# parthjaggi/flow

Measured on AMD Instinct MI355X. Metric: env-steps/sec, higher is better.
Workload: dtype mixed

## Files before the change

### flow_amd/build.py

```python
import concurrent.futures
import hashlib
import os
import shutil
import subprocess

PKG = os.path.dirname(os.path.abspath(__file__))
ROOT = os.path.dirname(PKG)
CSRC = os.path.join(PKG, "csrc")
SRC = os.path.join(CSRC, "flowsim.hip")
PART = os.path.join(CSRC, "flowsim_part.hip")
OBJ = os.path.join(CSRC, "_obj")
LIB = os.path.join(PKG, "libflowsim.so")

VALIDATED_ROCM = "7.2"

HEADERS = ["flowsim_sim.h", "flowsim_launch.h", "flowsim_kernels.h", "flowsim_open.h", "flowsim_wide.h",
           "flowsim_pair.h", "flowsim_pair_step_a.inc", "flowsim_pair_step_a_sm.inc", "flowsim_fig8.h", "flowsim_ringrl.h", "flowsim_policy.h", "flowsim_queue.h", "flowsim_queue_consts.h", "flowsim_dropq.h",
           "flowsim_learn.h",
           "flowsim_part.hip"]
DEPS = [SRC] + [os.path.join(CSRC, h) for h in HEADERS] + [os.path.join(ROOT, "include", "flowsim.h")]
assert all(os.path.exists(d) for d in DEPS)
_known = set(os.path.basename(d) for d in DEPS)
assert all(f in _known for f in os.listdir(CSRC) if f.endswith((".h", ".inc", ".hip"))), "flow_amd/build.py: a source under csrc/ is not in DEPS"

COMMON_FLAGS = ["--offload-arch=gfx950", "-O3", "-ffp-contract=off", "-std=c++17", "-Wall", "-Wno-unused-function"]
HIPCC_FLAGS = COMMON_FLAGS + ["-fPIC", "-shared"]


def parts():
    out = [("main", SRC, [])]
    for t, tn in (("float", "f32"), ("double", "f64")):
        for seg in (8, 16, 32, 64):
            out.append(("seg%d_%s" % (seg, tn), PART, ["-DFS_PART_T=" + t, "-DFS_PART_SEG=%d" % seg]))
        for w in (2, 4):
            out.append(("wide%d_%s" % (w, tn), PART, ["-DFS_PART_T=" + t, "-DFS_PART_WIDE=%d" % w]))
    out.append(("queue_f32", PART, ["-DFS_PART_T=float", "-DFS_PART_QUEUE=1"] +
                (["-DFS_QDIAG=1"] if os.environ.get("FLOWSIM_QDIAG") else [])))
    out.append(("learn_f32", PART, ["-DFS_PART_T=float", "-DFS_PART_LEARN=1"]))
    return out


def find_hipcc():
    for cand in (os.environ.get("HIPCC"), shutil.which("hipcc"), "/opt/rocm/bin/hipcc"):
        if cand and os.path.exists(cand):
            return cand
    raise RuntimeError("hipcc not found: libflowsim.so cannot be built (no CPU fallback exists)")


def include_flags():
    return ["-I" + os.path.join(ROOT, "include"), "-I" + CSRC]


def _stamp(extra):
    h = hashlib.sha256()
    for d in DEPS:
        h.update(os.path.relpath(d, ROOT).encode())
        with open(d, "rb") as f:
            h.update(hashlib.sha256(f.read()).digest())
# ... 158 lines not shown
```

### flow_amd/csrc/flowsim.hip

```cpp
#include "flowsim_sim.h"
#include "flowsim_learn.h"

namespace fsim {

int validate(const fs_config* c) {
  if (!c) return fail(FS_ERR_INVALID, "fs_create: cfg is NULL");
  if (c->struct_size != sizeof(fs_config))
    return fail(FS_ERR_INVALID, "fs_create: struct_size mismatch (header/library out of sync)");
  if (c->abi_version != FS_ABI_VERSION) return fail(FS_ERR_INVALID, "fs_create: abi_version mismatch");
  if (c->precision != FS_F32 && c->precision != FS_F64 && c->precision != FS_MIXED && c->precision != FS_F16S)
    return fail(FS_ERR_INVALID, "fs_create: bad precision");
  if (c->precision == FS_F16S && (c->network != FS_NET_MERGE || c->num_vehicles > 64))
    return fail(FS_ERR_UNSUPPORTED, "fs_create: FS_F16S (half state, float32 integrator) is built for FS_NET_MERGE "
                                    "(k_steps_open, <= 64 vehicle slots)");
  if (c->precision == FS_MIXED && (c->network == FS_NET_MERGE || c->network == FS_NET_BOTTLENECK)) {
  } else if (c->precision == FS_MIXED) {
    const bool fig8 = c->network == FS_NET_FIGURE_EIGHT;
    const char* why = nullptr;
    if ((c->network != FS_NET_RING && !fig8) || c->num_lanes > 1) why = "network (single-lane ring or figure eight)";
    else if (c->env != FS_ENV_ACCEL && c->env != FS_ENV_WAVE_ATTENUATION_PO) why = "env (AccelEnv or WaveAttenuationPOEnv)";
    else if (c->evaluate) why = "evaluate";
    else if (c->sims_per_step != 1) why = "sims_per_step (1)";
    else if (c->integrator != FS_EULER) why = "integrator (Euler)";
    else if (c->junction_mode && !fig8) why = "junction_mode";
// ... 214 lines not shown
    s->init_alive.assign(cfg->init_alive, cfg->init_alive + size_t(cfg->num_replicas) * cfg->num_vehicles);
    if (cfg->env == FS_ENV_BOTTLENECK_DV) {
      s->obs_cells.assign(cfg->obs_cells, cfg->obs_cells + cfg->num_obs_cells);
      if (cfg->num_rl > 0) s->act_cells.assign(cfg->act_cells, cfg->act_cells + cfg->num_rl);
    }
  }
  s->obs_dim = (cfg->env == FS_ENV_WAVE_ATTENUATION_PO) ? 3
               : (cfg->env == FS_ENV_WAVE_ATTENUATION_PO_MA) ? 3 * cfg->num_rl
               : (cfg->env == FS_ENV_ACCEL_PO_MA) ? 6 * cfg->num_rl
               : (cfg->env == FS_ENV_BOTTLENECK_DV) ? 4 * cfg->num_obs_cells + 1
               : (cfg->env == FS_ENV_BOTTLENECK) ? 1
               : (cfg->env == FS_ENV_MERGE_PO || cfg->env == FS_ENV_MERGE_MA)
                     ? 5 * cfg->num_rl
                     : (cfg->env == FS_ENV_LANE_CHANGE_ACCEL_PO)
                           ? (4 * (cfg->num_lanes < 1 ? 1 : cfg->num_lanes) + 1) * cfg->num_rl
                           : (cfg->env == FS_ENV_LANE_CHANGE_ACCEL ? 3 : 2) * cfg->num_vehicles;
  if (s->obs_dim < 1) s->obs_dim = 1;
  s->act_dim = cfg->num_rl * ((cfg->env == FS_ENV_LANE_CHANGE_ACCEL || cfg->env == FS_ENV_LANE_CHANGE_ACCEL_PO) ? 2 : 1);
  int seg = 8;
  while (seg < cfg->num_vehicles) seg <<= 1;
  s->seg = seg;
  hipError_t e = hipSetDevice(cfg->device);
  if (e == hipSuccess) e = hipStreamCreateWithFlags(&s->own_stream, hipStreamNonBlocking);
  if (e != hipSuccess) {
    delete s;
    return fail(FS_ERR_HIP, std::string("fs_create: no usable HIP device: ") + hipGetErrorString(e));
  }
  s->stream = s->own_stream;
  {
    const std::pair<const char*, bool SimBase::*> switches[] = {
        {"FLOWSIM_FORCE_GENERIC", &SimBase::force_generic}, {"FLOWSIM_NO_FASTDIV", &SimBase::no_fastdiv},
        {"FLOWSIM_NO_LOOP_KERNEL", &SimBase::no_loop_kernel}, {"FLOWSIM_NO_LOOP_FULL", &SimBase::no_loop_full},
        {"FLOWSIM_NO_RING_RL", &SimBase::no_ring_rl}, {"FLOWSIM_NO_QUEUE", &SimBase::no_queue},
        {"FLOWSIM_NO_PAIR", &SimBase::no_pair}, {"FLOWSIM_NO_MASK_SKIP", &SimBase::no_mask_skip}};
    for (const auto& sw : switches) {
      const char* v = std::getenv(sw.first);
      s->*sw.second = v && v[0] == '1';
    }
  }
  int rc = s->init();
  if (rc == FS_OK) {
    hipError_t e2 = hipStreamSynchronize(s->stream);
    if (e2 != hipSuccess) rc = fail(FS_ERR_HIP, std::string("fs_create: ") + hipGetErrorString(e2));
  }
  if (rc != FS_OK) {
    for (void* p : s->allocs) (void)hipFree(p);
    (void)hipStreamDestroy(s->own_stream);
    delete s;
    return rc;
  }
  s->cfg.vehicles = nullptr;
  s->cfg.ring_length = nullptr;
  s->cfg.init_pos = nullptr;
  s->cfg.init_vel = nullptr;
  s->cfg.init_lane = nullptr;
  s->cfg.segments = nullptr;
  s->cfg.inflows = nullptr;
  s->cfg.init_alive = nullptr;
  s->cfg.obs_cells = nullptr;
  s->cfg.obs_perm = nullptr;
  s->cfg.act_cells = nullptr;
  *out = reinterpret_cast<fs_handle>(static_cast<SimBase*>(s));
  return FS_OK;
}

inline SimBase* S(fs_handle h) { return reinterpret_cast<SimBase*>(h); }

// ... 338 lines not shown
```

### flow_amd/csrc/flowsim_kernels.h

```cpp
#pragma once
#include <hip/hip_runtime.h>
#include <stdint.h>

#include "flowsim.h"

namespace fs {

enum : int {
  FLAG_NEED_FOLLOWER = 1,
  FLAG_NEED_MEAN = 2,
  FLAG_HAS_NOISE = 4,
  FLAG_HAS_LAC = 8,
  FLAG_NEED_SUMO = 16,
  FLAG_HAS_FAILSAFE = 32,
  FLAG_ALL_IDM = 64,
  FLAG_IDM_SET = 128,
  FLAG_NO_FLOW_CTRL = 256,
  FLAG_DELTA4 = 512,
};

template <typename T>
struct DevView {
  T* pos;
  T* vel;
// ... 216 lines not shown
  T prv = dpp<DPP_WAVE_SHR1>(v);
  T last = v;
#pragma unroll
  for (int sg = 0; sg < 64 / SEG; ++sg) {
    T f = read_lane(v, sg * SEG + N - 1);
    last = (seg == sg) ? f : last;
  }
  return wrap ? last : prv;
}

template <int SEG, typename T>
__device__ __forceinline__ T seg_sum(T v) {
  v = v + dpp<DPP_QUAD_XOR1>(v);
  v = v + dpp<DPP_QUAD_XOR2>(v);
  v = v + dpp<DPP_ROW_HALF_MIRROR>(v);
  if (SEG >= 16) v = v + dpp<DPP_ROW_MIRROR>(v);
  if (SEG >= 32) v = add_swap16(v);
  if (SEG >= 64) v = add_swap32(v);
  return v;
}


template <int SHL, int SHR, typename T>
__device__ __forceinline__ T tr_combine(T lo, T hi, bool upper) {
  const T t = lo + dpp<SHL>(lo);
  const T u = hi + dpp<SHR>(hi);
  return upper ? u : t;
}
__device__ __forceinline__ float tr_combine16(float lo, float hi) {
  unsigned a = __builtin_bit_cast(unsigned, lo), b = __builtin_bit_cast(unsigned, hi);
  swap_rows16(a, b);
  return __builtin_bit_cast(float, a) + __builtin_bit_cast(float, b);
}
__device__ __forceinline__ double tr_combine16(double lo, double hi) {
  const unsigned long long bl = __builtin_bit_cast(unsigned long long, lo), bh = __builtin_bit_cast(unsigned long long, hi);
  unsigned l0 = unsigned(bl), l1 = unsigned(bl >> 32), h0 = unsigned(bh), h1 = unsigned(bh >> 32);
  swap_rows16(l0, h0);
  swap_rows16(l1, h1);
  return __builtin_bit_cast(double, ((unsigned long long)l1 << 32) | l0) +
         __builtin_bit_cast(double, ((unsigned long long)h1 << 32) | h0);
}
template <int SEG, int K, typename T>
__device__ __forceinline__ T transposed_sum(T* a, int lane) {
  static_assert(K <= 32 && K <= SEG, "at most min(SEG, 32) vectors");
  if (K >= 2) {
#pragma unroll
    for (int k = 0; k < K / 2; ++k) a[k] = tr_combine<DPP_ROW_SHL1, DPP_ROW_SHR1>(a[2 * k], a[2 * k + 1], (lane & 1) != 0);
  }
  if (K >= 4) {
#pragma unroll
    for (int k = 0; k < K / 4; ++k) a[k] = tr_combine<DPP_ROW_SHL2, DPP_ROW_SHR2>(a[2 * k], a[2 * k + 1], (lane & 2) != 0);
  }
  if (K >= 8) {
#pragma unroll
    for (int k = 0; k < K / 8; ++k) a[k] = tr_combine<DPP_ROW_SHL4, DPP_ROW_SHR4>(a[2 * k], a[2 * k + 1], (lane & 4) != 0);
  }
  if (K >= 16) {
#pragma unroll
    for (int k = 0; k < K / 16; ++k) a[k] = tr_combine<DPP_ROW_SHL8, DPP_ROW_SHR8>(a[2 * k], a[2 * k + 1], (lane & 8) != 0);
  }
  if (K >= 32) a[0] = tr_combine16(a[0], a[1]);
  T v = a[0];
  if (K < 2 && SEG >= 2) v = v + dpp<DPP_QUAD_XOR1>(v);
  if (K < 4 && SEG >= 4) v = v + dpp<DPP_QUAD_XOR2>(v);
  if (K < 8 && SEG >= 8) {
    if (K == 1) v = v + dpp<DPP_ROW_HALF_MIRROR>(v);
// ... 1446 lines not shown
```

### flow_amd/csrc/flowsim_launch.h

```cpp
#pragma once
#include "flowsim_sim.h"
#ifdef FS_PART_QUEUE
#include "flowsim_queue.h"
#include "flowsim_dropq.h"
#endif

namespace fsim {

#ifdef FS_PART_QUEUE
  template <typename T>
  int Sim<T>::launch_queue(const StepArgs& a) {
    const bool po = dv.env == FS_ENV_MERGE_PO;
    const bool noise = (dv.flags & fs::FLAG_HAS_NOISE) != 0, act = a.actions != nullptr && (po || ov.ma_apply_actions != 0);
    const auto k = pick(noise, [&](auto NZ) {
      return pick(act, [&](auto ACT) {
        return pick(po, [&](auto PO) { return &fs::k_merge_queue<NZ, ACT, false, PO>; });
      });
    });
    last_kernel = "k_merge_queue";
    hipLaunchKernelGGL(k, dim3(dv.R), dim3(64), 0, stream, dv, ov, qc, a.num_steps, a.actions, a.act_stride, a.obs, a.rew,
                       a.done, a.obs_every_step, fs::PolicyView{}, static_cast<float*>(nullptr), static_cast<float*>(nullptr),
                       0);
    return launched();
  }
// ... 202 lines not shown
                          : delta4 ? &fs::k_rollout_idm<T, SEG, true, false, BC> : &fs::k_rollout_idm<T, SEG, false, false, BC>;
    });
    last_kernel = "k_rollout_idm";
    const int waves = (dv.R + RPW - 1) / RPW;
    hipLaunchKernelGGL(k, dim3((waves + 7) / 8), dim3(512), 0, stream, dv, a.num_steps, a.obs, a.rew, a.done, d_dump);
    return launched();
  }

  template <typename T>
  template <int SEG>
  int Sim<T>::launch_k_steps(const StepArgs& a) {
    constexpr int RPW = 64 / SEG;
    auto k = &fs::k_steps<T, SEG, 0, 0>;
    last_kernel = "k_steps";
    if (fast_ok(a)) {
      k = &fs::k_steps<T, SEG, 1, 0>;
      last_kernel = "k_steps<FAST>";
    } else if ((dv.flags & fs::FLAG_IDM_SET) && !force_generic) {
      k = &fs::k_steps<T, SEG, 0, 1>;
      last_kernel = "k_steps<CSET>";
    }
    hipLaunchKernelGGL(k, dim3((dv.R + RPW - 1) / RPW), dim3(64), 0, stream, dv, a.num_steps, a.mask, a.actions,
                       a.act_stride, a.obs, a.rew, a.done, a.obs_every_step);
    return launched();
  }

  template <typename T>
  int Sim<T>::launch_policy_act(const fs::PolicyView& pv, int n_ag, const float* obs_in, float* act, float* logp) {
    last_kernel = "k_policy_act";
    const bool merge = dv.env == FS_ENV_MERGE_MA;
    hipLaunchKernelGGL(fs::k_policy_act<16>, dim3((dv.R * 16 + 255) / 256), dim3(256), 0, stream, pv, dv.R, n_ag, dv.rep0,
                       obs_in, act, logp, merge ? static_cast<const int*>(dv.lane) : nullptr,
                       merge ? static_cast<const int*>(dv.ctrl) : nullptr,
                       merge ? static_cast<const int*>(dv.rl_index) : nullptr, dv.N);
    return launched();
  }

  template <typename T>
  int Sim<T>::launch_policy_row16(const fs::PolicyView& pv, int num_steps, int reset_done, float* obs, float* act,
                                  float* logp, float* rew, uint8_t* done) {
    const bool fast = ringrl_fast_ok();
    auto kernel = [&](auto H) {
      return pick(dv.flags & fs::FLAG_HAS_NOISE, [&](auto NZ) {
        return pick(fast, [&](auto FA) { return &fs::k_ring_policy<T, H, NZ, FA>; });
      });
    };
    auto k = kernel(Int<1>());
    last_kernel = "k_ring_policy";
    if constexpr (std::is_same<T, float>::value) {
      if (dv.env == FS_ENV_WAVE_ATTENUATION_PO_MA) {
        k = kernel(Int<2>());
        last_kernel = "k_ring_policy<POMA>";
      }
    }
    const int waves = (dv.R + 3) / 4;
    hipLaunchKernelGGL(k, dim3((waves + 3) / 4), dim3(256), 0, stream, dv, pv, num_steps, reset_done, cfg.warmup_steps,
                       obs, act, logp, rew, done);
    return launched();
  }

  template <typename T>
  int Sim<T>::launch_policy_loop16(const fs::PolicyView& pv, int num_steps, int reset_done, float* obs, float* act,
                                   float* logp, float* rew, uint8_t* done) {
    if constexpr (std::is_same<T, float>::value) {
      const bool fastc = loop_delta4 && loop_fastc_ok();
      auto kernel = [&](auto H) {
        return fastc ? &fs::k_loop_policy<H, true, true>
// ... 16 lines not shown
```

### flow_amd/csrc/flowsim_policy.h

```cpp
#pragma once
#include "flowsim_ringrl.h"

namespace fs {

struct PolicyView {
  const float* w;
  const float* log_std;
  uint32_t* ctr;
  int in_dim, num_hidden, n_out;
  uint32_t seed_lo, seed_hi;
};

struct alignas(16) PolicyLds {
  float w_hid[2][16][16][4];
  float w_in[32][4];
  float w_wide[16][16][4];
  float b[3][32];
  float w_out[2][32];
  float b_out[2];
  float obs[4][4][4];
};

__host__ __device__ constexpr int policy_half(int in_dim) { return (in_dim + 1) >> 1; }

__device__ __forceinline__ void policy_wide_inputs(const float* o, int in_dim, int j, float& ia, float& ib) {
  const int half = policy_half(in_dim);
  ia = j < half ? o[j < half ? j : 0] : 0.0f;
  ib = (j < half && half + j < in_dim) ? o[half + j < in_dim ? half + j : 0] : 0.0f;
}

__device__ __forceinline__ const float* policy_load_trunk(const PolicyView& pv, PolicyLds* L, int tid, int nthreads) {
  const float* p = pv.w;
  const bool wide = pv.in_dim > 4;
  for (int e = tid; e < 32 * 4; e += nthreads) L->w_in[e / 4][e % 4] = (!wide && (e % 4) < pv.in_dim) ? p[(e / 4) * pv.in_dim + (e % 4)] : 0.0f;
  {
    const int half = policy_half(pv.in_dim);
    for (int e = tid; e < 32 * 32; e += nthreads) {
      const int u = e / 32, ip = e % 32;
      const int i = ip < 16 ? ip : half + (ip - 16);
      const bool used = wide && (ip & 15) < half && i < pv.in_dim;
      L->w_wide[ip >> 1][u & 15][(ip & 1) * 2 + (u >> 4)] = used ? p[u * pv.in_dim + i] : 0.0f;
    }
  }
  p += 32 * pv.in_dim;
  for (int e = tid; e < 32; e += nthreads) L->b[0][e] = p[e];
  p += 32;
  for (int l = 0; l < 2; ++l) {
    const bool have = l + 1 < pv.num_hidden;
    for (int e = tid; e < 32 * 32; e += nthreads) {
      const int u = e / 32, i = e % 32;
      L->w_hid[l][i >> 1][u & 15][(i & 1) * 2 + (u >> 4)] = have ? p[e] : 0.0f;
    }
    if (have) p += 32 * 32;
    for (int e = tid; e < 32; e += nthreads) L->b[l + 1][e] = have ? p[e] : 0.0f;
    if (have) p += 32;
  }
  return p;
}

__device__ __forceinline__ void policy_load(const PolicyView& pv, PolicyLds* L, int tid, int nthreads) {
  const float* p = policy_load_trunk(pv, L, tid, nthreads);
  for (int e = tid; e < 2 * 32; e += nthreads) L->w_out[e / 32][e % 32] = (e / 32) < pv.n_out ? p[e] : 0.0f;
  p += pv.n_out * 32;
  if (tid < 2) L->b_out[tid] = tid < pv.n_out ? p[tid] : 0.0f;
  __syncthreads();
}

template <int D1, int D2>
__device__ __forceinline__ void row_bcast(int k, float a, float b, float c, float& oa, float& ob, float& oc) {
#define FS_RB(K_) case K_: oa = dpp<DPP_ROW_NEWBCAST0 + K_>(a); ob = dpp<DPP_ROW_NEWBCAST0 + ((K_ + D1) & 15)>(b); \
                          oc = dpp<DPP_ROW_NEWBCAST0 + ((K_ + D2) & 15)>(c); break;
  switch (k & 15) {
    FS_RB(0) FS_RB(1) FS_RB(2) FS_RB(3) FS_RB(4) FS_RB(5) FS_RB(6) FS_RB(7)
    FS_RB(8) FS_RB(9) FS_RB(10) FS_RB(11) FS_RB(12) FS_RB(13) FS_RB(14) FS_RB(15)
  }
#undef FS_RB
}

__device__ __forceinline__ float policy_tanh(float z) {
  const float e = __builtin_amdgcn_exp2f(z * 2.885390081777927f);
  const float r = __builtin_amdgcn_rcpf(e + 1.0f);
  return __builtin_fmaf(-2.0f, r, 1.0f);
}

__device__ __forceinline__ f2 policy_layer(const float4 (&ww)[16], float b_j, float b_j16, float a, float b) {
  f2 z0 = {b_j, b_j16}, z1 = {0.0f, 0.0f}, z2 = {0.0f, 0.0f}, z3 = {0.0f, 0.0f};
  static_for<4>([&](auto q_c) {
    constexpr int q = decltype(q_c)::value;
    const float a0 = dpp<DPP_ROW_NEWBCAST0 + 4 * q>(a), a1 = dpp<DPP_ROW_NEWBCAST0 + 4 * q + 1>(a);
    const float a2 = dpp<DPP_ROW_NEWBCAST0 + 4 * q + 2>(a), a3 = dpp<DPP_ROW_NEWBCAST0 + 4 * q + 3>(a);
    const float b0 = dpp<DPP_ROW_NEWBCAST0 + 4 * q>(b), b1 = dpp<DPP_ROW_NEWBCAST0 + 4 * q + 1>(b);
    const float b2 = dpp<DPP_ROW_NEWBCAST0 + 4 * q + 2>(b), b3 = dpp<DPP_ROW_NEWBCAST0 + 4 * q + 3>(b);
    z0 = fma2(f2{ww[2 * q].x, ww[2 * q].y}, splat(a0), z0);
    z1 = fma2(f2{ww[2 * q].z, ww[2 * q].w}, splat(a1), z1);
    z2 = fma2(f2{ww[2 * q + 1].x, ww[2 * q + 1].y}, splat(a2), z2);
    z3 = fma2(f2{ww[2 * q + 1].z, ww[2 * q + 1].w}, splat(a3), z3);
    z0 = fma2(f2{ww[8 + 2 * q].x, ww[8 + 2 * q].y}, splat(b0), z0);
    z1 = fma2(f2{ww[8 + 2 * q].z, ww[8 + 2 * q].w}, splat(b1), z1);
    z2 = fma2(f2{ww[8 + 2 * q + 1].x, ww[8 + 2 * q + 1].y}, splat(b2), z2);
    z3 = fma2(f2{ww[8 + 2 * q + 1].z, ww[8 + 2 * q + 1].w}, splat(b3), z3);
  });
  return pk_add(pk_add(z0, z1), pk_add(z2, z3));
}

template <bool WIDE, bool PRE = false>
__device__ __forceinline__ void policy_trunk(const PolicyView& pv, const PolicyLds* L, int j, float o0, float o1, float o2,
                                             float& ha, float& hb) {
  float4 wa0 = make_float4(0.0f, 0.0f, 0.0f, 0.0f), wa1 = wa0;
  auto load_ahead = [&](int l) {
    wa0 = *reinterpret_cast<const float4*>(L->w_hid[l][0][j]);
    wa1 = *reinterpret_cast<const float4*>(L->w_hid[l][1][j]);
  };
  if (pv.num_hidden > 1) load_ahead(0);
  if constexpr (PRE) {
    ha = policy_tanh(o0);
    hb = policy_tanh(o1);
  } else if constexpr (WIDE) {
    float4 ww[16];
#pragma unroll
    for (int q = 0; q < 16; ++q) ww[q] = *reinterpret_cast<const float4*>(L->w_wide[q][j]);
    const f2 z = policy_layer(ww, L->b[0][j], L->b[0][j + 16], o0, o1);
    ha = policy_tanh(z.x);
    hb = policy_tanh(z.y);
  } else {
    const float4 wa = *reinterpret_cast<const float4*>(L->w_in[j]), wb = *reinterpret_cast<const float4*>(L->w_in[j + 16]);
    float za = L->b[0][j], zb = L->b[0][j + 16];
    za = __builtin_fmaf(wa.x, o0, za); zb = __builtin_fmaf(wb.x, o0, zb);
    za = __builtin_fmaf(wa.y, o1, za); zb = __builtin_fmaf(wb.y, o1, zb);
    za = __builtin_fmaf(wa.z, o2, za); zb = __builtin_fmaf(wb.z, o2, zb);
    ha = policy_tanh(za);
    hb = policy_tanh(zb);
  }
#pragma unroll 1
  for (int l = 0; l + 1 < pv.num_hidden; ++l) {
    float4 ww[16];
    ww[0] = wa0;
    ww[1] = wa1;
#pragma unroll
    for (int q = 2; q < 16; ++q) ww[q] = *reinterpret_cast<const float4*>(L->w_hid[l][q][j]);
    const f2 z = policy_layer(ww, L->b[l + 1][j], L->b[l + 1][j + 16], ha, hb);
    if (l + 2 < pv.num_hidden) load_ahead(l + 1);
    ha = policy_tanh(z.x);
    hb = policy_tanh(z.y);
  }
}

template <int ROW, bool WIDE = false>
__device__ __forceinline__ void policy_eval(const PolicyView& pv, const PolicyLds* L, int j, float o0, float o1, float o2,
                                            float& mu, float& log_std) {
  static_assert(ROW == 16, "policy_eval: a row of 16 lanes holds the 32 units of a layer");
  float ha, hb;
  policy_trunk<WIDE>(pv, L, j, o0, o1, o2, ha, hb);
  float p0 = L->w_out[0][j] * ha, p1 = L->w_out[1][j] * ha;
  p0 = __builtin_fmaf(L->w_out[0][j + 16], hb, p0);
  p1 = __builtin_fmaf(L->w_out[1][j + 16], hb, p1);
  mu = seg_sum<ROW>(p0) + L->b_out[0];
  const float o1_ = seg_sum<ROW>(p1) + L->b_out[1];
  log_std = pv.log_std != nullptr ? pv.log_std[0] : o1_;
}

__device__ __forceinline__ void policy_sample(const PolicyView& pv, uint32_t replica, uint32_t ctr, float mu, float log_std,
                                              float& action, float& logp, NoiseBlock<float>* nzb = nullptr,
                                              uint32_t agent = 0u) {
  const uint32_t col = 0x40000000u + agent;
  const float g = nzb ? nzb->draw(pv.seed_lo, pv.seed_hi, replica, col, ctr)
                      : gauss<float>(pv.seed_lo, pv.seed_hi, replica, col, ctr);
  const float sd = __builtin_amdgcn_exp2f(log_std * 1.4426950408889634f);
  action = __builtin_fmaf(sd, g, mu);
  logp = __builtin_fmaf(-0.5f * g, g, -log_std) - 0.9189385332046727f;
}

__device__ __forceinline__ void policy_sample_agent(const PolicyView& pv, uint32_t replica, uint32_t ctr, int c, float mu,
                                                    float log_std, float& action, float& logp, NoiseBlock<float>& nzb0,
                                                    NoiseBlock<float>& nzb1) {
  if (c == 0) policy_sample(pv, replica, ctr, mu, log_std, action, logp, &nzb0, 0u);
  else if (c == 1) policy_sample(pv, replica, ctr, mu, log_std, action, logp, &nzb1, 1u);
  else policy_sample(pv, replica, ctr, mu, log_std, action, logp, nullptr, uint32_t(c));
}

__device__ __forceinline__ float policy_no_action() { return __builtin_nanf(""); }

template <int ROW>
__device__ __forceinline__ unsigned long long policy_present(const int* slot_lane, const int* slot_ctrl,
                                                             const int* slot_rl, int N, int rr, int j) {
  if (slot_lane == nullptr) return ~0ull;
  unsigned lo = 0u, hi = 0u;
  for (int i = j; i < N; i += ROW) {
    if (slot_ctrl[i] != FS_CTRL_RL || slot_lane[size_t(rr) * N + i] < 0) continue;
    const int c = slot_rl[i] & 63;
    lo |= c < 32 ? 1u << c : 0u;
    hi |= c >= 32 ? 1u << (c - 32) : 0u;
  }
  return (static_cast<unsigned long long>(seg_or<ROW>(hi)) << 32) | seg_or<ROW>(lo);
}

template <int ROW>
__global__ __launch_bounds__(256) void k_policy_act(PolicyView pv, int R, int n_ag, uint32_t rep0,
                                                    const float* __restrict__ obs, float* __restrict__ act,
                                                    float* __restrict__ logp, const int* __restrict__ slot_lane,
                                                    const int* __restrict__ slot_ctrl, const int* __restrict__ slot_rl,
                                                    int N) {
  __shared__ PolicyLds L;
  policy_load(pv, &L, threadIdx.x, blockDim.x);
  const int lane = threadIdx.x & 63, j = lane & 15;
  const int r = (blockIdx.x * blockDim.x + threadIdx.x) >> 4;
  const int rr = r < R ? r : R - 1;
  const uint32_t c0 = pv.ctr[rr];
  const unsigned long long present = policy_present<ROW>(slot_lane, slot_ctrl, slot_rl, N, rr, j);
#pragma unroll 1
  for (int c = 0; c < n_ag; ++c) {
    const float* o = obs + (size_t(rr) * n_ag + c) * pv.in_dim;
    float mu, ls;
    if (pv.in_dim > 4) {
      float ia, ib;
      policy_wide_inputs(o, pv.in_dim, j, ia, ib);
      policy_eval<ROW, true>(pv, &L, j, ia, ib, 0.0f, mu, ls);
    } else {
      policy_eval<ROW>(pv, &L, j, o[0], pv.in_dim > 1 ? o[1] : 0.0f, pv.in_dim > 2 ? o[2] : 0.0f, mu, ls);
    }
    float a, lp;
    policy_sample(pv, rep0 + uint32_t(rr), c0, mu, ls, a, lp, nullptr, uint32_t(c));
    if (r < R && j == 0) {
      const bool here = ((present >> (c & 63)) & 1ull) != 0ull;
      act[size_t(r) * n_ag + c] = here ? a : policy_no_action();
      logp[size_t(r) * n_ag + c] = here ? lp : 0.0f;
    }
  }
  if (r < R && j == 0) pv.ctr[r] = c0 + 1u;
}

constexpr int FS_POLICY_VEC_MAX = 6;

struct alignas(16) PolicyVecLds {
  float w_out[2 * FS_POLICY_VEC_MAX][32];
  float b_out[2 * FS_POLICY_VEC_MAX];
  float log_std[FS_POLICY_VEC_MAX];
  float lp[16];
};

__device__ __forceinline__ void policy_vec_load(const PolicyView& pv, int A, PolicyLds* L, PolicyVecLds* V, int tid,
                                                int nthreads) {
  const float* p = policy_load_trunk(pv, L, tid, nthreads);
  const int n_out = pv.n_out;
  for (int e = tid; e < 2 * FS_POLICY_VEC_MAX * 32; e += nthreads) V->w_out[e / 32][e % 32] = (e / 32) < n_out ? p[e] : 0.0f;
  for (int e = tid; e < 2 * FS_POLICY_VEC_MAX; e += nthreads) V->b_out[e] = e < n_out ? p[n_out * 32 + e] : 0.0f;
  for (int e = tid; e < FS_POLICY_VEC_MAX; e += nthreads) V->log_std[e] = (pv.log_std != nullptr && e < A) ? pv.log_std[e] : 0.0f;
  __syncthreads();
}

__device__ __forceinline__ float policy_vec_act(const PolicyView& pv, int A, const PolicyLds* L, PolicyVecLds* V,
                                                uint32_t replica, uint32_t ctr, int lane, const float* o, float* act_row,
// ... 152 lines not shown
template <int ROW>
__global__ __launch_bounds__(256) void k_policy_act_wide(PolicyView pv, int R, int A, uint32_t rep0,
                                                         const float* __restrict__ obs, float* __restrict__ act,
                                                         float* __restrict__ logp) {
  static_assert(ROW == 16, "k_policy_act_wide: a row of 16 lanes holds the 32 units of a layer");
  __shared__ PolicyLds L;
  __shared__ PolicyWideLds W;
  const float* w_out = policy_load_trunk(pv, &L, threadIdx.x, blockDim.x);
  __syncthreads();
  const int lane = threadIdx.x & 63, wave = threadIdx.x >> 6;
  const int r = blockIdx.x * 4 + wave;
  if (r >= R) return;
  const uint32_t c0 = pv.ctr[r];
  float a;
  const float lp = policy_wide_act(pv, A, &L, w_out, W.lp[wave], rep0 + uint32_t(r), c0, lane, obs + size_t(r) * pv.in_dim, a);
  if (lane < A) act[size_t(r) * A + lane] = a;
  if (lane == 0) {
    logp[r] = lp;
    pv.ctr[r] = c0 + 1u;
  }
}

template <typename T, int HEAD, bool NOISE, bool FAST>
__global__ __launch_bounds__(256) void k_ring_policy(DevView<T> s, PolicyView pv, int num_steps, int reset_done,
                                                     int warmup_steps, float* __restrict__ obs, float* __restrict__ act,
                                                     float* __restrict__ logp, float* __restrict__ rew,
                                                     uint8_t* __restrict__ done) {
  constexpr int ROW = 16;
  constexpr bool MIXED = sizeof(T) == 8;
  constexpr bool MA = HEAD == 2;
  static_assert(HEAD == 1 || HEAD == 2, "k_ring_policy: the PO heads");
  static_assert(!(MA && MIXED), "the multi-agent head exists in float32 only");
  __shared__ PolicyLds PL;
  policy_load(pv, &PL, threadIdx.x, blockDim.x);
  RingPairCore<T, ROW, NOISE, FAST> core(s);
  const int lane = core.lane, k = core.k, N = core.N, LP = core.LP, rr = core.rr, iA = core.iA, iB = core.iB;
  const bool rvalid = core.rvalid, valid = core.valid, last = core.last, rlA = core.rlA, rlB = core.rlB;
  uint32_t pctr = pv.ctr[rr];
  core.set_length(s.ring_len[rr] + T(4) * s.jlen);
  core.load_state(s.pos, s.vel);
  core.snapshot();
  const f2 &v = core.v, &vl = core.vl, &h = core.h, &dgap = core.dgap;

  const bool poA = valid && rlA, poB = valid && rlB;
  const double rc15 = 1.0 / 15.0, pml64 = double(s.po_max_length), rc_pml64 = 1.0 / pml64;
  float o0 = 0.0f, o1 = 0.0f, o2 = 0.0f;
  auto observe_po = [&](int k_rl, bool selB, float third, float* orow) {
    const float v_me = selB ? v.y : v.x, v_ld = selB ? vl.y : vl.x;
    const float n1 = dpp<0x120 + 1>(v_ld - v_me), n2 = dpp<0x120 + 2>(third);
    const int pc = (k - k_rl) & (ROW - 1);
    const float n = pc == 0 ? v_me : (pc == 1 ? n1 : n2);
    const float q = div_via_f64(n, pc == 2 ? pml64 : 15.0, pc == 2 ? rc_pml64 : rc15);
    if (rvalid && pc < 3) orow[pc] = q;
    row_bcast<1, 2>(k_rl, q, q, q, o0, o1, o2);
  };
  const unsigned long long po_m = __ballot(poA || poB);
  const int k_po = po_m ? (__builtin_ctzll(po_m) & (ROW - 1)) : 0;
  const int src0 = (lane - k) + k_po;
  auto observe = [&](float* orow) {
    if constexpr (!MIXED && ROW == 16) {
      observe_po(k_po, poB, poB ? dgap.y : dgap.x, orow);
    } else {
      float q0, q1, q2;
      if (MIXED) {
        const double vdn = next_a<ROW>(core.vdA, last, lane);
        const double v_me = poB ? core.vdB : core.vdA, v_ld = poB ? vdn : core.vdB, d_me = poB ? core.dgB : core.dgA;
        q0 = float(v_me * rc15);
// ... 12 lines not shown
      }
      o0 = __shfl(q0, src0, 64);
      o1 = __shfl(q1, src0, 64);
      o2 = __shfl(q2, src0, 64);
    }
  };

  const int n_ag = MA ? s.num_rl : 1;
  const int colA = rlA ? s.rl_index[iA] : -1, colB = rlB ? s.rl_index[iB] : -1;
  const bool redA = MA && valid && iA < s.num_rl, redB = MA && valid && iB < s.num_rl;
  const int obs_dim = MA ? 3 * n_ag : 3;
  auto observe_agent = [&](int c, float* orow) {
    const unsigned long long m = __ballot(k < LP && (colA == c || colB == c));
    const int k_c = m ? (__builtin_ctzll(m) & (ROW - 1)) : 0;
    observe_po(k_c, colB == c, colB == c ? h.y : h.x, orow + 3 * c);
  };

  const size_t R = size_t(s.R);
  NoiseBlock<float> act_draws, act_draws1;
  act_draws.init();
  act_draws1.init();
  if constexpr (!MA) observe(obs + size_t(rr) * 3);
  for (int step = 0; step < num_steps; ++step) {
    float a, aA, aB, arA = 0.0f, arB = 0.0f;
    if constexpr (MA) {
      aA = 0.0f;
      aB = 0.0f;
      a = 0.0f;
      float* orow = obs + (size_t(step) * R + rr) * obs_dim;
#pragma unroll 1
      for (int c = 0; c < n_ag; ++c) {
        observe_agent(c, orow);
        float mu, ls, ac, lp;
        policy_eval<ROW>(pv, &PL, k, o0, o1, o2, mu, ls);
        policy_sample_agent(pv, s.rep0 + uint32_t(rr), pctr, c, mu, ls, ac, lp, act_draws, act_draws1);
        if (rvalid && k == 0) {
          act[(size_t(step) * R + rr) * n_ag + c] = ac;
          logp[(size_t(step) * R + rr) * n_ag + c] = lp;
        }
        aA = colA == c ? ac : aA;
        aB = colB == c ? ac : aB;
        arA = iA == c ? ac : arA;
        arB = iB == c ? ac : arB;
      }
    } else {
      float mu, ls, lp;
      policy_eval<ROW>(pv, &PL, k, o0, o1, o2, mu, ls);
      policy_sample(pv, s.rep0 + uint32_t(rr), pctr, mu, ls, a, lp, &act_draws);
      if (rvalid && k == 0) {
        act[size_t(step) * R + rr] = a;
        logp[size_t(step) * R + rr] = lp;
      }
      aA = a;
      aB = a;
    }
    pctr += 1u;
    core.template advance<false>(true, true, aA, aB);
    const unsigned fany = seg_or<ROW>(core.step_flags());
    const bool crashed = !MA && (fany & 1u) != 0u;
    const bool bad = (fany & 2u) != 0u || crashed;
    const float sv = seg_sum<ROW>(valid ? v.x + v.y : 0.0f);
    float mean_a;
    if constexpr (MA) {
      const float caA = tabs(core.clip(arA)), caB = tabs(core.clip(arB));
      const float sa = seg_sum<ROW>((redA ? caA : 0.0f) + (redB ? caB : 0.0f));
      mean_a = div_via_f64(sa, double(s.num_rl), 1.0 / double(s.num_rl));
    } else {
      mean_a = tabs(core.clip(a));
    }
    const float reward = wave_reward(sv, N, mean_a, bad);
    const uint8_t dflag = done_flag(core.tcount >= s.step_limit, crashed);
    if (rvalid && k == 0) {
      rew[size_t(step) * R + rr] = reward;
      done[size_t(step) * R + rr] = dflag;
    }
    const bool fin = reset_done && dflag != 0;
    if (__ballot(fin) != 0ull) {
      if (fin) {
        core.load_state(s.init_pos, s.init_vel);
        core.set_length(s.init_ring_len[rr] + T(4) * s.jlen);
        core.tcount = 0;
      }
      core.snapshot();
#pragma unroll 1
      for (int w = 0; w < warmup_steps; ++w) core.template advance<false>(fin, false, 0.0f, 0.0f);
      if (fin && valid && core.kk == 0) const_cast<T*>(s.ring_len)[rr] = s.init_ring_len[rr];
    }
    if constexpr (!MA) observe(obs + (size_t(step + 1) * R + rr) * 3);
  }
  if constexpr (MA) {
#pragma unroll 1
    for (int c = 0; c < n_ag; ++c) observe_agent(c, obs + (size_t(num_steps) * R + rr) * obs_dim);
  }

  if (valid) {
    core.store_state();
    if (core.kk == 0) pv.ctr[rr] = pctr;
  }
}


template <int HEAD, bool DELTA4, bool FASTC>
__global__ __launch_bounds__(256) void k_loop_policy(DevView<float> s, PolicyView pv, int num_steps, int reset_done,
                                                     float* __restrict__ obs, float* __restrict__ act,
                                                     float* __restrict__ logp, float* __restrict__ rew,
                                                     uint8_t* __restrict__ done) {
  typedef float T;
  typedef float X;
  constexpr int SEG = 16, RPW = 4;
  __shared__ X tab_start[FS_MAX_SEGMENTS + 2], tab_fs[FS_MAX_SEGMENTS + 2], tab_sl[FS_MAX_SEGMENTS + 2];
  __shared__ PolicyLds PL;
  policy_load(pv, &PL, threadIdx.x, blockDim.x);
  const int lane = threadIdx.x & 63;
  const int wave = (blockIdx.x * blockDim.x + threadIdx.x) >> 6;
  const int seg = lane / SEG;
  const int i = lane % SEG;
  const int r = wave * RPW + seg;
  const int N = s.N;
  const bool rvalid = r < s.R;
  const bool valid = rvalid && i < N;
  const int rr = rvalid ? r : s.R - 1;
  const int ii = i < N ? i : N - 1;
  const size_t idx = size_t(rr) * N + ii;
  const bool wrap_lead = (i + 1 >= N);
  constexpr bool has = true;
  const int flags = s.flags;

  if (threadIdx.x < FS_MAX_SEGMENTS + 2) {
    const int q = threadIdx.x, qq = q < FS_MAX_SEGMENTS ? q : 0;
    tab_start[q] = q < s.nseg ? s.seg_start[qq] : X(3.0e38);
    tab_fs[q] = q < s.nseg ? s.seg_flow_start[qq] : X(0);
    tab_sl[q] = q < s.nseg ? s.seg_flow_slope[qq] : X(0);
  }
  __syncthreads();

  Slot<T> sl;
  sl.ctrl = s.ctrl[ii];
  sl.failsafe = 0;
  sl.speed_mode = s.speed_mode[ii];
  sl.rl_index = s.rl_index[ii];
  sl.pis_index = -1;
#pragma unroll
  for (int k = 0; k < FS_MAX_CTRL_PARAMS; ++k) sl.p[k] = T(s.p[k * N + ii]);
  sl.noise = T(s.noise[ii]);
  sl.delay = T(0);
// ... 102 lines not shown
      const float po0 = divc(v, d_15), po1 = divc(vl - v, d_15), po2 = divc(d, d_po);
      if (obs_lane) { orow[0] = po0; orow[1] = po1; orow[2] = po2; }
      row_bcast<0, 0>(k_rl, po0, po1, po2, o0, o1, o2);
    } else {
      const X xo = c_fs + c_sl * (x - c_st);
      const float po0 = divc(v, d_ms), po1 = divc(xo, d_L);
      if (obs_lane) { orow[ii] = po0; orow[N + ii] = po1; }
      o0 = valid ? po0 : 0.0f;
      o1 = valid ? po1 : 0.0f;
    }
  };

  const size_t R = size_t(s.R);
  const int n_ag = HEAD == 2 ? num_rl : 1;
  NoiseBlock<float> act_draws, act_draws1;
  act_draws.init();
  act_draws1.init();
  observe(obs + size_t(rr) * obs_dim);
  for (int step = 0; step < num_steps; ++step) {
    float mu, ls, a, lp;
    if constexpr (HEAD == 2) {
      a = 0.0f;
#pragma unroll 1
      for (int c = 0; c < n_ag; ++c) {
        const unsigned long long m = __ballot(i < N && rl_lane && sl.rl_index == c);
        const int i_c = m ? (__builtin_ctzll(m) & (SEG - 1)) : 0;
        const int f_c = i_c == 0 ? N - 1 : i_c - 1;
        float a0, a1, a2, b0, b1, b2;
        row_bcast<0, 0>(i_c, m0, m1, m2, a0, a1, a2);
        row_bcast<0, 0>(f_c, m3l, m2, m5, b0, b1, b2);
        const float ia = i == 0 ? a0 : (i == 1 ? a1 : (i == 2 ? a2 : 0.0f));
        const float ib = i == 0 ? b0 : (i == 1 ? b1 : (i == 2 ? b2 : 0.0f));
        float ac;
        policy_eval<SEG, true>(pv, &PL, i, ia, ib, 0.0f, mu, ls);
        policy_sample_agent(pv, s.rep0 + uint32_t(rr), pctr, c, mu, ls, ac, lp, act_draws, act_draws1);
        if (rvalid && i == 0) {
          act[(size_t(step) * R + rr) * n_ag + c] = ac;
          logp[(size_t(step) * R + rr) * n_ag + c] = lp;
        }
        a = (rl_lane && own_col == c) ? ac : a;
      }
    } else {
      if (HEAD == 1) policy_eval<SEG>(pv, &PL, i, o0, o1, o2, mu, ls);
      else policy_eval<SEG, true>(pv, &PL, i, o0, o1, 0.0f, mu, ls);
      policy_sample(pv, s.rep0 + uint32_t(rr), pctr, mu, ls, a, lp, &act_draws);
      if (rvalid && i == 0) {
        act[size_t(step) * R + rr] = a;
        logp[size_t(step) * R + rr] = lp;
      }
    }
    pctr += 1u;
    bool on_a = false, on_b = false, on_any = false, on_both = false;
    if (junction_on) {
      const unsigned on_b_m = sm_in(x, jb_in - look, jb_in) & (jf << 31);
      const unsigned on_a_m = sm_in(x, ja_in - look, ja_in) & (jf << 30);
      on_b = sm_true(on_b_m);
      on_a = sm_true(on_a_m);
      on_any = sm_true(on_a_m | on_b_m);
      on_both = sm_true(on_a_m & on_b_m);
    }
    const unsigned on_edge_u = 1u ^ (gate_u & (seg_internal >> k));
    const unsigned commanded_u = (on_edge_u & cmd_other) | cmd_rl;
    const bool commanded = commanded_u != 0u;
    T acc;
    {
      if (any_noise) {
        if (__ballot(noisy && (nctr & 3u) == 0u) != 0ull) {
          if (noisy && (nctr & 3u) == 0u)
            gauss4<T>(s.seed_lo, s.seed_hi, s.rep0 + uint32_t(rr), uint32_t(ii), nctr >> 2, g4, s.noise_exact != 0);
        }
      }
      T ai = idm_fast<DELTA4, FASTC>(T(v), T(vl), h, has, ic);
      if (any_noise) {
        const T an = ai + sl.noise * g4[0];
        ai = noisy ? an : ai;
        g4[0] = g4[1]; g4[1] = g4[2]; g4[2] = g4[3];
      }
// ... 99 lines not shown
```

### flow_amd/csrc/flowsim_sim.h

```cpp
#pragma once
#include <hip/hip_runtime.h>

#include <algorithm>
#include <climits>
#include <cmath>
#include <cstdio>
#include <cstdlib>
#include <cstring>
#include <map>
#include <mutex>
#include <new>
#include <string>
#include <type_traits>
#include <vector>

#include "flowsim.h"
#include "flowsim_kernels.h"
#include "flowsim_open.h"
#include "flowsim_pair.h"
#include "flowsim_fig8.h"
#include "flowsim_ringrl.h"
#include "flowsim_policy.h"
#include "flowsim_wide.h"
#include "flowsim_queue_consts.h"
// ... 36 lines not shown

struct SimBase {
  virtual ~SimBase() {}
  fs_config cfg{};
  std::vector<fs_vehicle_spec> veh;
  std::vector<fs_segment> segs;
  std::vector<fs_inflow> inflows;
  std::vector<fs_cell> obs_cells, act_cells;
  std::vector<int32_t> obs_perm;
  std::vector<uint8_t> init_alive;
  int obs_dim = 0;
  int act_dim = 0;
  int seg = 0;
  hipStream_t own_stream = nullptr;
  hipStream_t stream = nullptr;
  float* d_actions = nullptr;
  float* d_obs = nullptr;
  float* d_rew = nullptr;
  uint8_t* d_done = nullptr;
  uint8_t* d_mask = nullptr;
  float* d_dump = nullptr;
  std::vector<void*> allocs;
  int after_reset = 0;
  bool force_generic = false;
  bool no_fastdiv = false;
  bool f16s = false;
  bool mixed = false;
  bool no_pair = false;
  bool no_loop_kernel = false;
  bool no_loop_full = false;
  bool no_ring_rl = false;
  bool no_mask_skip = false;
  bool no_queue = false;
  double* d_adv_scratch = nullptr;
  int* d_qflag = nullptr;
  bool qflag_armed = false;
  int check_qflag() {
    if (!qflag_armed || !d_qflag) return FS_OK;
    int f = 0;
    HIP_TRY(hipMemcpy(&f, d_qflag, sizeof(int), hipMemcpyDeviceToHost));
    if (f != 0)
      return fail(FS_ERR_UNSUPPORTED, "k_drop_queue: a path of the lane-drop network held more than 64 vehicles (or more than 8 "
                                      "arrived in one sub-step): the results of this handle are invalid -- create it "
                                      "with FLOWSIM_NO_QUEUE=1 (slot-order kernels)");
    qflag_armed = false;
    return FS_OK;
  }
  bool has_user_ctrl = false;
  const char* last_kernel = "";
  int launched() {
    HIP_TRY(hipGetLastError());
    return FS_OK;
  }

  virtual int launch_steps(int num_steps, const uint8_t* mask, const float* actions, size_t act_stride,
                           float* obs, float* rew, uint8_t* done, int obs_every_step) = 0;
  virtual int launch_reset(const uint8_t* mask) = 0;
  virtual int launch_policy(const fs_policy* pol, int num_steps, int reset_done, const float* obs_in, float* obs,
                            float* act, float* logp, float* rew, uint8_t* done) = 0;
  uint32_t* d_pol_ctr = nullptr;
  virtual int get_state(int field, void* dst, size_t bytes) = 0;
  virtual int set_state(int field, const void* src, size_t bytes) = 0;
  virtual int add_vehicle(int replica, int slot, int route, double x, double speed) = 0;
};

template <typename T>
// ... 1072 lines not shown
```

Baseline: 13.47 billion.

## Evaluate policy MLP hidden layers with 4x4x1 f32 MFMA instead of LDS FMAs

```diff
diff --git a/flow_amd/build.py b/flow_amd/build.py
--- a/flow_amd/build.py
+++ b/flow_amd/build.py
@@ -23,7 +23,8 @@
 _known = set(os.path.basename(d) for d in DEPS)
 assert all(f in _known for f in os.listdir(CSRC) if f.endswith((".h", ".inc", ".hip"))), "flow_amd/build.py: a source under csrc/ is not in DEPS"
 
-COMMON_FLAGS = ["--offload-arch=gfx950", "-O3", "-ffp-contract=off", "-std=c++17", "-Wall", "-Wno-unused-function"]
+COMMON_FLAGS = ["--offload-arch=gfx950", "-O3", "-ffp-contract=off", "-std=c++17", "-Wall", "-Wno-unused-function",
+                "-mllvm", "-amdgpu-mfma-vgpr-form"]
 HIPCC_FLAGS = COMMON_FLAGS + ["-fPIC", "-shared"]
 
 
diff --git a/flow_amd/csrc/flowsim.hip b/flow_amd/csrc/flowsim.hip
--- a/flow_amd/csrc/flowsim.hip
+++ b/flow_amd/csrc/flowsim.hip
@@ -270,7 +270,8 @@
         {"FLOWSIM_FORCE_GENERIC", &SimBase::force_generic}, {"FLOWSIM_NO_FASTDIV", &SimBase::no_fastdiv},
         {"FLOWSIM_NO_LOOP_KERNEL", &SimBase::no_loop_kernel}, {"FLOWSIM_NO_LOOP_FULL", &SimBase::no_loop_full},
         {"FLOWSIM_NO_RING_RL", &SimBase::no_ring_rl}, {"FLOWSIM_NO_QUEUE", &SimBase::no_queue},
-        {"FLOWSIM_NO_PAIR", &SimBase::no_pair}, {"FLOWSIM_NO_MASK_SKIP", &SimBase::no_mask_skip}};
+        {"FLOWSIM_NO_PAIR", &SimBase::no_pair}, {"FLOWSIM_NO_MASK_SKIP", &SimBase::no_mask_skip},
+        {"FLOWSIM_POLICY_LDS", &SimBase::policy_lds}};
     for (const auto& sw : switches) {
       const char* v = std::getenv(sw.first);
       s->*sw.second = v && v[0] == '1';
diff --git a/flow_amd/csrc/flowsim_kernels.h b/flow_amd/csrc/flowsim_kernels.h
--- a/flow_amd/csrc/flowsim_kernels.h
+++ b/flow_amd/csrc/flowsim_kernels.h
@@ -272,6 +272,11 @@
   swap_rows16(a, b);
   return __builtin_bit_cast(float, a) + __builtin_bit_cast(float, b);
 }
+__device__ __forceinline__ float tr_combine32(float lo, float hi) {
+  unsigned a = __builtin_bit_cast(unsigned, lo), b = __builtin_bit_cast(unsigned, hi);
+  swap_rows32(a, b);
+  return __builtin_bit_cast(float, a) + __builtin_bit_cast(float, b);
+}
 __device__ __forceinline__ double tr_combine16(double lo, double hi) {
   const unsigned long long bl = __builtin_bit_cast(unsigned long long, lo), bh = __builtin_bit_cast(unsigned long long, hi);
   unsigned l0 = unsigned(bl), l1 = unsigned(bl >> 32), h0 = unsigned(bh), h1 = unsigned(bh >> 32);
diff --git a/flow_amd/csrc/flowsim_launch.h b/flow_amd/csrc/flowsim_launch.h
--- a/flow_amd/csrc/flowsim_launch.h
+++ b/flow_amd/csrc/flowsim_launch.h
@@ -258,7 +258,7 @@
     hipLaunchKernelGGL(fs::k_policy_act<16>, dim3((dv.R * 16 + 255) / 256), dim3(256), 0, stream, pv, dv.R, n_ag, dv.rep0,
                        obs_in, act, logp, merge ? static_cast<const int*>(dv.lane) : nullptr,
                        merge ? static_cast<const int*>(dv.ctrl) : nullptr,
-                       merge ? static_cast<const int*>(dv.rl_index) : nullptr, dv.N);
+                       merge ? static_cast<const int*>(dv.rl_index) : nullptr, dv.N, policy_lds ? 0 : 1);
     return launched();
   }
 
diff --git a/flow_amd/csrc/flowsim_policy.h b/flow_amd/csrc/flowsim_policy.h
--- a/flow_amd/csrc/flowsim_policy.h
+++ b/flow_amd/csrc/flowsim_policy.h
@@ -29,17 +29,29 @@
   ib = (j < half && half + j < in_dim) ? o[half + j < in_dim ? half + j : 0] : 0.0f;
 }
 
-__device__ __forceinline__ const float* policy_load_trunk(const PolicyView& pv, PolicyLds* L, int tid, int nthreads) {
+__device__ __forceinline__ void policy_b_place(int e, int& u, int& ip) {
+  const int c = e & 3, ln = (e >> 2) & 63, t = e >> 8;
+  u = (ln & 15) + 16 * (c & 1);
+  ip = 16 * (c >> 1) + 4 * t + (ln >> 4);
+}
+
+__device__ __forceinline__ const float* policy_load_trunk(const PolicyView& pv, PolicyLds* L, int tid, int nthreads,
+                                                          bool mfma = false) {
   const float* p = pv.w;
   const bool wide = pv.in_dim > 4;
   for (int e = tid; e < 32 * 4; e += nthreads) L->w_in[e / 4][e % 4] = (!wide && (e % 4) < pv.in_dim) ? p[(e / 4) * pv.in_dim + (e % 4)] : 0.0f;
   {
     const int half = policy_half(pv.in_dim);
     for (int e = tid; e < 32 * 32; e += nthreads) {
-      const int u = e / 32, ip = e % 32;
+      int u = e / 32, ip = e % 32;
+      float* dst = &L->w_wide[ip >> 1][u & 15][(ip & 1) * 2 + (u >> 4)];
+      if (mfma) {
+        policy_b_place(e, u, ip);
+        dst = &L->w_wide[0][0][0] + e;
+      }
       const int i = ip < 16 ? ip : half + (ip - 16);
       const bool used = wide && (ip & 15) < half && i < pv.in_dim;
-      L->w_wide[ip >> 1][u & 15][(ip & 1) * 2 + (u >> 4)] = used ? p[u * pv.in_dim + i] : 0.0f;
+      *dst = used ? p[u * pv.in_dim + i] : 0.0f;
     }
   }
   p += 32 * pv.in_dim;
@@ -48,8 +60,13 @@
   for (int l = 0; l < 2; ++l) {
     const bool have = l + 1 < pv.num_hidden;
     for (int e = tid; e < 32 * 32; e += nthreads) {
-      const int u = e / 32, i = e % 32;
-      L->w_hid[l][i >> 1][u & 15][(i & 1) * 2 + (u >> 4)] = have ? p[e] : 0.0f;
+      int u = e / 32, i = e % 32;
+      float* dst = &L->w_hid[l][i >> 1][u & 15][(i & 1) * 2 + (u >> 4)];
+      if (mfma) {
+        policy_b_place(e, u, i);
+        dst = &L->w_hid[l][0][0][0] + e;
+      }
+      *dst = have ? p[u * 32 + i] : 0.0f;
     }
     if (have) p += 32 * 32;
     for (int e = tid; e < 32; e += nthreads) L->b[l + 1][e] = have ? p[e] : 0.0f;
@@ -58,8 +75,8 @@
   return p;
 }
 
-__device__ __forceinline__ void policy_load(const PolicyView& pv, PolicyLds* L, int tid, int nthreads) {
-  const float* p = policy_load_trunk(pv, L, tid, nthreads);
+__device__ __forceinline__ void policy_load(const PolicyView& pv, PolicyLds* L, int tid, int nthreads, bool mfma = false) {
+  const float* p = policy_load_trunk(pv, L, tid, nthreads, mfma);
   for (int e = tid; e < 2 * 32; e += nthreads) L->w_out[e / 32][e % 32] = (e / 32) < pv.n_out ? p[e] : 0.0f;
   p += pv.n_out * 32;
   if (tid < 2) L->b_out[tid] = tid < pv.n_out ? p[tid] : 0.0f;
@@ -103,18 +120,59 @@
   return pk_add(pk_add(z0, z1), pk_add(z2, z3));
 }
 
-template <bool WIDE, bool PRE = false>
-__device__ __forceinline__ void policy_trunk(const PolicyView& pv, const PolicyLds* L, int j, float o0, float o1, float o2,
-                                             float& ha, float& hb) {
+typedef float f4 __attribute__((ext_vector_type(4)));
+__device__ __forceinline__ f2 policy_layer_mfma(const float4 (&wb)[4], float b_j, float b_j16, float a, float b, int lane) {
+  const int src = ((lane & 3) << 6) | ((lane >> 4) << 2);
+  float in[8];
+  static_for<4>([&](auto q_c) {
+    constexpr int q = decltype(q_c)::value;
+    in[2 * q] = __builtin_bit_cast(float, __builtin_amdgcn_ds_bpermute(src + 16 * q, __builtin_bit_cast(int, a)));
+    in[2 * q + 1] = __builtin_bit_cast(float, __builtin_amdgcn_ds_bpermute(src + 16 * q, __builtin_bit_cast(int, b)));
+  });
+  __builtin_amdgcn_sched_barrier(0);
+  const float c_j = lane < 16 ? b_j : 0.0f, c_j16 = lane < 16 ? b_j16 : 0.0f;
+  f4 za = {c_j, c_j, c_j, c_j}, zb = {c_j16, c_j16, c_j16, c_j16};
+  static_for<4>([&](auto q_c) {
+    constexpr int q = decltype(q_c)::value;
+    za = __builtin_amdgcn_mfma_f32_4x4x1f32(in[2 * q], wb[q].x, za, 0, 0, 0);
+    zb = __builtin_amdgcn_mfma_f32_4x4x1f32(in[2 * q], wb[q].y, zb, 0, 0, 0);
+    za = __builtin_amdgcn_mfma_f32_4x4x1f32(in[2 * q + 1], wb[q].z, za, 0, 0, 0);
+    zb = __builtin_amdgcn_mfma_f32_4x4x1f32(in[2 * q + 1], wb[q].w, zb, 0, 0, 0);
+  });
+  return f2{tr_combine32(tr_combine16(za[0], za[1]), tr_combine16(za[2], za[3])),
+            tr_combine32(tr_combine16(zb[0], zb[1]), tr_combine16(zb[2], zb[3]))};
+}
+
+template <bool WIDE, bool PRE, bool MFMA>
+__device__ __forceinline__ void policy_trunk_form(const PolicyView& pv, const PolicyLds* L, int j, float o0, float o1,
+                                                  float o2, float& ha, float& hb) {
+  static_assert(!(MFMA && PRE), "policy_wide_layer1's rows are not four evaluations of one network");
+  int lane = threadIdx.x & 63;
+  if constexpr (MFMA) asm volatile("" : "+v"(lane), "+v"(j));
+  float4 wb[4];
+  auto load_b = [&](const float* w) {
+#pragma unroll
+    for (int t = 0; t < 4; ++t) wb[t] = *reinterpret_cast<const float4*>(w + (t * 64 + lane) * 4);
+  };
+  auto layer_mfma = [&](const float* bias, float a, float b) {
+    return policy_layer_mfma(wb, bias[j], bias[j + 16], a, b, lane);
+  };
   float4 wa0 = make_float4(0.0f, 0.0f, 0.0f, 0.0f), wa1 = wa0;
   auto load_ahead = [&](int l) {
     wa0 = *reinterpret_cast<const float4*>(L->w_hid[l][0][j]);
     wa1 = *reinterpret_cast<const float4*>(L->w_hid[l][1][j]);
   };
-  if (pv.num_hidden > 1) load_ahead(0);
+  if constexpr (!MFMA) {
+    if (pv.num_hidden > 1) load_ahead(0);
+  }
   if constexpr (PRE) {
     ha = policy_tanh(o0);
     hb = policy_tanh(o1);
+  } else if constexpr (WIDE && MFMA) {
+    load_b(&L->w_wide[0][0][0]);
+    const f2 z = layer_mfma(L->b[0], o0, o1);
+    ha = policy_tanh(z.x);
+    hb = policy_tanh(z.y);
   } else if constexpr (WIDE) {
     float4 ww[16];
 #pragma unroll
@@ -123,34 +181,52 @@
     ha = policy_tanh(z.x);
     hb = policy_tanh(z.y);
   } else {
-    const float4 wa = *reinterpret_cast<const float4*>(L->w_in[j]), wb = *reinterpret_cast<const float4*>(L->w_in[j + 16]);
+    const float4 wa = *reinterpret_cast<const float4*>(L->w_in[j]), wc = *reinterpret_cast<const float4*>(L->w_in[j + 16]);
     float za = L->b[0][j], zb = L->b[0][j + 16];
-    za = __builtin_fmaf(wa.x, o0, za); zb = __builtin_fmaf(wb.x, o0, zb);
-    za = __builtin_fmaf(wa.y, o1, za); zb = __builtin_fmaf(wb.y, o1, zb);
-    za = __builtin_fmaf(wa.z, o2, za); zb = __builtin_fmaf(wb.z, o2, zb);
+    za = __builtin_fmaf(wa.x, o0, za); zb = __builtin_fmaf(wc.x, o0, zb);
+    za = __builtin_fmaf(wa.y, o1, za); zb = __builtin_fmaf(wc.y, o1, zb);
+    za = __builtin_fmaf(wa.z, o2, za); zb = __builtin_fmaf(wc.z, o2, zb);
     ha = policy_tanh(za);
     hb = policy_tanh(zb);
   }
 #pragma unroll 1
   for (int l = 0; l + 1 < pv.num_hidden; ++l) {
-    float4 ww[16];
-    ww[0] = wa0;
-    ww[1] = wa1;
+    if constexpr (MFMA) {
+      load_b(&L->w_hid[l][0][0][0]);
+      const f2 z = layer_mfma(L->b[l + 1], ha, hb);
+      ha = policy_tanh(z.x);
+      hb = policy_tanh(z.y);
+    } else {
+      float4 ww[16];
+      ww[0] = wa0;
+      ww[1] = wa1;
 #pragma unroll
-    for (int q = 2; q < 16; ++q) ww[q] = *reinterpret_cast<const float4*>(L->w_hid[l][q][j]);
-    const f2 z = policy_layer(ww, L->b[l + 1][j], L->b[l + 1][j + 16], ha, hb);
-    if (l + 2 < pv.num_hidden) load_ahead(l + 1);
-    ha = policy_tanh(z.x);
-    hb = policy_tanh(z.y);
+      for (int q = 2; q < 16; ++q) ww[q] = *reinterpret_cast<const float4*>(L->w_hid[l][q][j]);
+      const f2 z = policy_layer(ww, L->b[l + 1][j], L->b[l + 1][j + 16], ha, hb);
+      if (l + 2 < pv.num_hidden) load_ahead(l + 1);
+      ha = policy_tanh(z.x);
+      hb = policy_tanh(z.y);
+    }
+  }
+}
+
+template <bool WIDE, bool PRE = false>
+__device__ __forceinline__ void policy_trunk(const PolicyView& pv, const PolicyLds* L, int j, float o0, float o1, float o2,
+                                             float& ha, float& hb, bool mfma = false) {
+  if constexpr (PRE) {
+    policy_trunk_form<WIDE, PRE, false>(pv, L, j, o0, o1, o2, ha, hb);
+  } else {
+    if (mfma) policy_trunk_form<WIDE, PRE, true>(pv, L, j, o0, o1, o2, ha, hb);
+    else policy_trunk_form<WIDE, PRE, false>(pv, L, j, o0, o1, o2, ha, hb);
   }
 }
 
 template <int ROW, bool WIDE = false>
 __device__ __forceinline__ void policy_eval(const PolicyView& pv, const PolicyLds* L, int j, float o0, float o1, float o2,
-                                            float& mu, float& log_std) {
+                                            float& mu, float& log_std, bool mfma = false) {
   static_assert(ROW == 16, "policy_eval: a row of 16 lanes holds the 32 units of a layer");
   float ha, hb;
-  policy_trunk<WIDE>(pv, L, j, o0, o1, o2, ha, hb);
+  policy_trunk<WIDE>(pv, L, j, o0, o1, o2, ha, hb, mfma);
   float p0 = L->w_out[0][j] * ha, p1 = L->w_out[1][j] * ha;
   p0 = __builtin_fmaf(L->w_out[0][j + 16], hb, p0);
   p1 = __builtin_fmaf(L->w_out[1][j + 16], hb, p1);
@@ -199,9 +275,10 @@
                                                     const float* __restrict__ obs, float* __restrict__ act,
                                                     float* __restrict__ logp, const int* __restrict__ slot_lane,
                                                     const int* __restrict__ slot_ctrl, const int* __restrict__ slot_rl,
-                                                    int N) {
+                                                    int N, int mfma_form) {
   __shared__ PolicyLds L;
-  policy_load(pv, &L, threadIdx.x, blockDim.x);
+  const bool mfma = mfma_form != 0;
+  policy_load(pv, &L, threadIdx.x, blockDim.x, mfma);
   const int lane = threadIdx.x & 63, j = lane & 15;
   const int r = (blockIdx.x * blockDim.x + threadIdx.x) >> 4;
   const int rr = r < R ? r : R - 1;
@@ -214,9 +291,9 @@
     if (pv.in_dim > 4) {
       float ia, ib;
       policy_wide_inputs(o, pv.in_dim, j, ia, ib);
-      policy_eval<ROW, true>(pv, &L, j, ia, ib, 0.0f, mu, ls);
+      policy_eval<ROW, true>(pv, &L, j, ia, ib, 0.0f, mu, ls, mfma);
     } else {
-      policy_eval<ROW>(pv, &L, j, o[0], pv.in_dim > 1 ? o[1] : 0.0f, pv.in_dim > 2 ? o[2] : 0.0f, mu, ls);
+      policy_eval<ROW>(pv, &L, j, o[0], pv.in_dim > 1 ? o[1] : 0.0f, pv.in_dim > 2 ? o[2] : 0.0f, mu, ls, mfma);
     }
     float a, lp;
     policy_sample(pv, rep0 + uint32_t(rr), c0, mu, ls, a, lp, nullptr, uint32_t(c));
@@ -435,7 +512,8 @@
   static_assert(HEAD == 1 || HEAD == 2, "k_ring_policy: the PO heads");
   static_assert(!(MA && MIXED), "the multi-agent head exists in float32 only");
   __shared__ PolicyLds PL;
-  policy_load(pv, &PL, threadIdx.x, blockDim.x);
+  constexpr bool mfma = true;
+  policy_load(pv, &PL, threadIdx.x, blockDim.x, mfma);
   RingPairCore<T, ROW, NOISE, FAST> core(s);
   const int lane = core.lane, k = core.k, N = core.N, LP = core.LP, rr = core.rr, iA = core.iA, iB = core.iB;
   const bool rvalid = core.rvalid, valid = core.valid, last = core.last, rlA = core.rlA, rlB = core.rlB;
@@ -514,7 +592,7 @@
       for (int c = 0; c < n_ag; ++c) {
         observe_agent(c, orow);
         float mu, ls, ac, lp;
-        policy_eval<ROW>(pv, &PL, k, o0, o1, o2, mu, ls);
+        policy_eval<ROW>(pv, &PL, k, o0, o1, o2, mu, ls, mfma);
         policy_sample_agent(pv, s.rep0 + uint32_t(rr), pctr, c, mu, ls, ac, lp, act_draws, act_draws1);
         if (rvalid && k == 0) {
           act[(size_t(step) * R + rr) * n_ag + c] = ac;
@@ -527,7 +605,7 @@
       }
     } else {
       float mu, ls, lp;
-      policy_eval<ROW>(pv, &PL, k, o0, o1, o2, mu, ls);
+      policy_eval<ROW>(pv, &PL, k, o0, o1, o2, mu, ls, mfma);
       policy_sample(pv, s.rep0 + uint32_t(rr), pctr, mu, ls, a, lp, &act_draws);
       if (rvalid && k == 0) {
         act[size_t(step) * R + rr] = a;
@@ -592,7 +670,8 @@
   constexpr int SEG = 16, RPW = 4;
   __shared__ X tab_start[FS_MAX_SEGMENTS + 2], tab_fs[FS_MAX_SEGMENTS + 2], tab_sl[FS_MAX_SEGMENTS + 2];
   __shared__ PolicyLds PL;
-  policy_load(pv, &PL, threadIdx.x, blockDim.x);
+  constexpr bool mfma = true;
+  policy_load(pv, &PL, threadIdx.x, blockDim.x, mfma);
   const int lane = threadIdx.x & 63;
   const int wave = (blockIdx.x * blockDim.x + threadIdx.x) >> 6;
   const int seg = lane / SEG;
@@ -761,7 +840,7 @@
         const float ia = i == 0 ? a0 : (i == 1 ? a1 : (i == 2 ? a2 : 0.0f));
         const float ib = i == 0 ? b0 : (i == 1 ? b1 : (i == 2 ? b2 : 0.0f));
         float ac;
-        policy_eval<SEG, true>(pv, &PL, i, ia, ib, 0.0f, mu, ls);
+        policy_eval<SEG, true>(pv, &PL, i, ia, ib, 0.0f, mu, ls, mfma);
         policy_sample_agent(pv, s.rep0 + uint32_t(rr), pctr, c, mu, ls, ac, lp, act_draws, act_draws1);
         if (rvalid && i == 0) {
           act[(size_t(step) * R + rr) * n_ag + c] = ac;
@@ -770,8 +849,8 @@
         a = (rl_lane && own_col == c) ? ac : a;
       }
     } else {
-      if (HEAD == 1) policy_eval<SEG>(pv, &PL, i, o0, o1, o2, mu, ls);
-      else policy_eval<SEG, true>(pv, &PL, i, o0, o1, 0.0f, mu, ls);
+      if (HEAD == 1) policy_eval<SEG>(pv, &PL, i, o0, o1, o2, mu, ls, mfma);
+      else policy_eval<SEG, true>(pv, &PL, i, o0, o1, 0.0f, mu, ls, mfma);
       policy_sample(pv, s.rep0 + uint32_t(rr), pctr, mu, ls, a, lp, &act_draws);
       if (rvalid && i == 0) {
         act[size_t(step) * R + rr] = a;
diff --git a/flow_amd/csrc/flowsim_sim.h b/flow_amd/csrc/flowsim_sim.h
--- a/flow_amd/csrc/flowsim_sim.h
+++ b/flow_amd/csrc/flowsim_sim.h
@@ -92,6 +92,7 @@
   bool no_ring_rl = false;
   bool no_mask_skip = false;
   bool no_queue = false;
+  bool policy_lds = false;
   double* d_adv_scratch = nullptr;
   int* d_qflag = nullptr;
   bool qflag_armed = false;
```

Result: no change. 13.54 billion, median of 5 (+0.5%).
